# leeyevi/MV3D_TF

Hardware: AMD Instinct MI355X
Metric: KITTI-shape frames/sec (RPN+3-view ROI-pool+NMS) at 1/2/4/8 MI355X (higher is better)
Workload: dtype f32; 1 GPU; BASELINE configs[2] path-only: batch 2, 3 views; proposal_layer_3d TRAIN cfg (23104 BEV anchors, pre/post-NMS 12000/2000, NMS 0.7) + anchor_target + proposal_target (256 sampled ROIs in batch 0) + FV ROIs + RoiPool 7x7 fwd+bwd on BEV 76x76x512 / RGB 46x155x512 / FV 8x64x512; peaky scores; driven by the library's own mv3d_train_path (submit -> counts to the host -> numpy-global-RNG draws on the hel; batch_per_gpu=2, ring_batches=16, streams=8, launch=path, hipgraph=False, parallelism=frames/1, pmc_signature=train/b2/r256/peaky/pair-tiles-planned

## Files before the change

### include/mv3d_hip.h

```cpp
#ifndef MV3D_HIP_H
#define MV3D_HIP_H
#include <stddef.h>
#include <stdint.h>
#ifdef __cplusplus
extern "C" {
#endif

typedef enum {
    MV3D_OK = 0,
    MV3D_ERR_INVALID_ARG = 1,
    MV3D_ERR_WORKSPACE = 2,
    MV3D_ERR_HIP = 3,
    MV3D_ERR_ZERO_DIVISION = 4
} mv3d_status;

int mv3d_version(void);
const char *mv3d_status_string(int status);


size_t mv3d_nms_workspace_bytes(int max_boxes);
int mv3d_nms_device(const float *dets_dev, int n, double thresh, int max_keep,
                    int32_t *keep_dev, int32_t *num_keep_dev, int32_t *status_dev,
                    void *workspace, size_t workspace_bytes, void *stream);

// ... 103 lines not shown
                              const int32_t *disable_bg2_dev, int n_dis_bg2,
                              float *labels_dev, float *anchors_dev, float *anchors_3d_dev,
                              int32_t *n_anchors_dev, int anchors_cap,
                              void *workspace, size_t workspace_bytes, void *stream);

int mv3d_anchor_target_stage1_batch(int batch, int H, int W, const float *im_info_dev, const float *const *gt_bv_dev,
                                    const float *const *gt_3d_dev, const int *G, const mv3d_anchor_target_params *p,
                                    float *labels_dev, float *targets_dev, int32_t *const *counts_dev,
                                    uint8_t *const *fg_hi_dev, void *const *workspace, size_t workspace_bytes, void *stream);
int mv3d_anchor_target_stage2_batch(int batch, int H, int W, const mv3d_anchor_target_params *p,
                                    const int32_t *const *disable_fg_dev, const int *n_dis_fg,
                                    const int32_t *const *disable_bg1_dev, const int *n_dis_bg1,
                                    const int32_t *const *disable_bg2_dev, const int *n_dis_bg2, float *labels_dev,
                                    float *anchors_dev, float *anchors_3d_dev, int32_t *n_anchors_dev, int anchors_cap,
                                    void *const *workspace, size_t workspace_bytes, void *stream);

typedef struct {
    int32_t num_classes;
    int32_t frame_index;
    double fg_thresh;
    double bg_thresh_hi;
    double bg_thresh_lo;
} mv3d_proposal_target_params;

size_t mv3d_proposal_target_workspace_bytes(int num_rois, int G);
int mv3d_proposal_target_stage1(const float *rois_bv_dev, const float *rois_3d_dev, int num_rois,
                                const float *gt_bv_dev, const float *gt_3d_dev, int G,
                                const mv3d_proposal_target_params *p, int32_t *counts_dev,
                                void *workspace, size_t workspace_bytes, void *stream);
int mv3d_proposal_target_stage2(const float *rois_bv_dev, const float *rois_3d_dev, int num_rois,
// ... 43 lines not shown
int mv3d_legacy_permutation(void *mt19937_state, int32_t n, int32_t *out);
typedef struct {
    int32_t n_fg, n_bg, n_low;
    int32_t pt_n_fg, pt_n_bg;
    int32_t reserved0;
    const uint8_t *fg_alive;
} mv3d_draw_frame;
typedef struct {
    int32_t rpn_batchsize;
    int32_t rpn_num_fg;
    int32_t rois_per_image;
    int32_t roi_fg_max;
} mv3d_draw_params;
int mv3d_draw_training_subsamples(void *mt19937_state, int batch, const mv3d_draw_frame *frames, const mv3d_draw_params *par,
                                  int32_t *lists, size_t lists_cap, int32_t *sizes, int32_t *scratch, size_t scratch_cap);

typedef struct {
    int32_t batch, H, W, num_classes;
    int32_t proposal_cap;
    int32_t anchor_cap;
    int32_t roi_cap;
    int32_t max_gt;
    mv3d_proposal_params proposal;
    mv3d_anchor_target_params anchor;
    mv3d_proposal_target_params target;
    mv3d_draw_params draw;
} mv3d_train_path_config;
typedef struct {
    float *blob_bv, *blob_img, *blob_3d;
    int32_t *num_proposals;
// ... 11 lines not shown
    uint8_t *h_report; size_t h_report_row;
    int32_t *h_pt_counts;
    int32_t *h_num_proposals;
    int32_t *h_lists;
    int32_t *h_scratch; size_t scratch_cap;
} mv3d_train_path_slot;
typedef struct mv3d_train_path mv3d_train_path;
int mv3d_train_path_create(const mv3d_train_path_config *config, int depth, const mv3d_train_path_slot *slots, int helper_thread,
                           mv3d_train_path **out);
int mv3d_train_path_configure(mv3d_train_path *path, const mv3d_train_path_config *config);
int mv3d_train_path_submit(mv3d_train_path *path, int slot, const float *prob_dev, const float *pred_dev, const float *im_info_dev,
                           const float *calib_dev, const float *const *gt_bv_dev, const float *const *gt_3d_dev,
                           const float *const *gt_corners_dev, const int *G, void *mt19937_state, void *stream);
int mv3d_train_path_finish(mv3d_train_path *path, int slot, int32_t *rows_out, int32_t *num_proposals_out, int32_t *sizes_out);
int mv3d_train_path_host_seconds(mv3d_train_path *path, double *wait_s, double *draw_s);
void mv3d_train_path_destroy(mv3d_train_path *path);

int mv3d_gt_encode(const float *box_cam_dev, const double *cos_sin_dev, int num_objects, const float *inv_rot_dev,
                   const float *tr_velo_to_cam_dev, float *corners_cam_dev, float *corners_lidar_dev,
                   float *boxes_3d_dev, float *boxes_bv_dev, void *stream);

int mv3d_box_detect_tail(const float *rois_3d_dev, const float *bbox_pred_dev, int num_rois, int num_classes,
                         float *corners_dev, float *pred_cnr_r_dev, float *pred_bv_dev, float *pred_bv_r_dev,
                         void *stream);

typedef struct {
    int32_t num_classes;
    int32_t rows_per_frame;
    int32_t max_per_image;
    int32_t nms_strict_gt;
// ... 195 lines not shown
```

### mv3d_tf_amd/_lib.py

```python
import ctypes as C
import os

import torch

_HERE = os.path.dirname(os.path.abspath(__file__))
LIB_PATH = os.path.join(_HERE, "libmv3d_hip.so")

OK, ERR_INVALID_ARG, ERR_WORKSPACE, ERR_HIP, ERR_ZERO_DIVISION = 0, 1, 2, 3, 4


class ProposalParams(C.Structure):
    _fields_ = [("feat_stride", C.c_int32), ("pre_nms_topN", C.c_int32), ("post_nms_topN", C.c_int32),
                ("img_height", C.c_int32), ("img_width", C.c_int32), ("img_padding", C.c_int32),
                ("nms_strict_gt", C.c_int32), ("reserved0", C.c_int32), ("nms_thresh", C.c_double), ("min_size", C.c_double)]


class DetectPostParams(C.Structure):
    _fields_ = [("num_classes", C.c_int32), ("rows_per_frame", C.c_int32), ("max_per_image", C.c_int32),
                ("nms_strict_gt", C.c_int32), ("score_thresh", C.c_float), ("reserved0", C.c_int32), ("nms_thresh", C.c_double)]


class AnchorTargetParams(C.Structure):
    _fields_ = [("feat_stride", C.c_int32), ("clobber_positives", C.c_int32),
                ("negative_overlap", C.c_double), ("positive_overlap", C.c_double)]
# ... 109 lines not shown
    "mv3d_proposal_3d": (C.c_int, [_P, _P, C.c_int, C.c_int, C.c_int, _P, _P, C.POINTER(ProposalParams),
                                   _P, _P, _P, _P, _P, _P, C.c_size_t, _P]),
    "mv3d_roi_pool_forward": (C.c_int, [_P, C.c_float, C.c_int, C.c_int, C.c_int, C.c_int, C.c_int, C.c_int,
                                        C.c_int, _P, _P, _P, _P]),
    "mv3d_roi_pool_backward": (C.c_int, [_P, C.c_float, C.c_int, C.c_int, C.c_int, C.c_int, C.c_int, C.c_int,
                                         C.c_int, _P, _P, _P, _P]),
    "mv3d_anchor_target_workspace_bytes": (C.c_size_t, [C.c_int, C.c_int, C.c_int]),
    "mv3d_anchor_target_stage1": (C.c_int, [C.c_int, C.c_int, _P, _P, _P, C.c_int, C.POINTER(AnchorTargetParams),
                                            _P, _P, _P, _P, _P, C.c_size_t, _P]),
    "mv3d_anchor_target_stage2": (C.c_int, [C.c_int, C.c_int, C.POINTER(AnchorTargetParams), _P, C.c_int, _P,
                                            C.c_int, _P, C.c_int, _P, _P, _P, _P, C.c_int, _P, C.c_size_t, _P]),
    "mv3d_anchor_target_stage1_batch": (C.c_int, [C.c_int, C.c_int, C.c_int, _P, _P, _P, _P, C.POINTER(AnchorTargetParams), _P, _P, _P, _P,
                                                  _P, C.c_size_t, _P]),
    "mv3d_anchor_target_stage2_batch": (C.c_int, [C.c_int, C.c_int, C.c_int, C.POINTER(AnchorTargetParams), _P, _P, _P, _P, _P, _P, _P,
                                                  _P, _P, _P, C.c_int, _P, C.c_size_t, _P]),
    "mv3d_proposal_target_stage1_batch": (C.c_int, [C.c_int, _P, _P, _P, _P, _P, _P, _P, _P, _P, _P, _P]),
    "mv3d_proposal_target_stage2_batch": (C.c_int, [C.c_int, _P, _P, _P, _P, _P, _P, _P, _P, _P, _P, _P, _P, _P, _P, _P, _P, _P, _P, _P,
                                                    _P, _P, _P]),
    "mv3d_proposal_target_stage1_batch_devn": (C.c_int, [C.c_int, _P, _P, _P, _P, _P, _P, _P, _P, _P, _P, _P, _P]),
    "mv3d_proposal_target_stage2_batch_devn": (C.c_int, [C.c_int, _P, _P, _P, _P, _P, _P, _P, _P, _P, _P, _P, _P, _P, _P, _P, _P, _P, _P,
                                                         _P, _P, _P, _P, _P]),
    "mv3d_proposal_target_workspace_bytes": (C.c_size_t, [C.c_int, C.c_int]),
    "mv3d_proposal_target_stage1": (C.c_int, [_P, _P, C.c_int, _P, _P, C.c_int, C.POINTER(ProposalTargetParams), _P, _P,
                                              C.c_size_t, _P]),
    "mv3d_proposal_target_stage2": (C.c_int, [_P, _P, C.c_int, _P, _P, _P, C.c_int, _P, C.POINTER(ProposalTargetParams),
                                              _P, C.c_int, _P, C.c_int, _P, _P, _P, _P, _P, _P, C.c_size_t, _P]),
    "mv3d_point_cloud_2_top": (C.c_int, [_P, C.c_int, _P, _P]),
    "mv3d_point_cloud_2_top_shape": (C.c_int, [C.c_double] * 8 + [_P]),
    "mv3d_point_cloud_2_top_ranges": (C.c_int, [_P, C.c_int] + [C.c_double] * 8 + [_P, _P, _P]),
    "mv3d_box_detect_tail": (C.c_int, [_P, _P, C.c_int, C.c_int, _P, _P, _P, _P, _P]),
# ... 9 lines not shown
    "mv3d_roi_pool_forward_views": (C.c_int, [C.c_int, C.POINTER(RoiView), C.c_int, C.c_int, _P]),
    "mv3d_roi_pool_forward_views_cold": (C.c_int, [C.c_int, C.POINTER(RoiView), C.c_int, C.c_int, _P]),
    "mv3d_roi_pool_forward_views_half": (C.c_int, [C.c_int, C.POINTER(RoiView), C.c_int, C.c_int, C.c_int, C.c_int, _P]),
    "mv3d_roi_pool_backward_workspace_bytes": (C.c_size_t, [C.c_int, C.POINTER(RoiGradView), C.c_int, C.c_int]),
    "mv3d_roi_pool_backward_views": (C.c_int, [C.c_int, C.POINTER(RoiGradView), C.c_int, C.c_int, _P, C.c_size_t, _P]),
    "mv3d_roi_pool_pair_workspace_bytes": (C.c_size_t, [C.c_int, C.POINTER(RoiGradView), C.c_int, C.c_int]),
    "mv3d_roi_pool_forward_views_pair": (C.c_int, [C.c_int, C.POINTER(RoiView), C.c_int, C.c_int, C.c_int, _P]),
    "mv3d_roi_pool_backward_views_pair": (C.c_int, [C.c_int, C.POINTER(RoiGradView), C.c_int, C.c_int, _P, C.c_size_t, _P]),
    "mv3d_roi_pool_argmax_decode": (C.c_int, [C.c_int, C.POINTER(RoiView), C.c_int, C.c_int, C.POINTER(C.c_void_p), _P]),
    "mv3d_ROIPoolForwardLaucher": (C.c_int, [_P, C.c_float, C.c_int, C.c_int, C.c_int, C.c_int, C.c_int, C.c_int, _P, _P, _P, _P]),
    "mv3d_ROIPoolBackwardLaucher": (C.c_int, [_P, C.c_float, C.c_int, C.c_int, C.c_int, C.c_int, C.c_int, C.c_int, C.c_int, _P, _P, _P, _P]),
    "mv3d_rois_3d_to_fv": (C.c_int, [_P, C.c_int, _P, _P]),
    "mv3d_legacy_permutation": (C.c_int, [_P, C.c_int32, _P]),
    "mv3d_draw_training_subsamples": (C.c_int, [_P, C.c_int, C.POINTER(DrawFrame), C.POINTER(DrawParams), _P, C.c_size_t, _P, _P,
                                                C.c_size_t]),
    "mv3d_train_path_create": (C.c_int, [C.POINTER(TrainPathConfig), C.c_int, C.POINTER(TrainPathSlot), C.c_int, C.POINTER(C.c_void_p)]),
    "mv3d_train_path_configure": (C.c_int, [_P, C.POINTER(TrainPathConfig)]),
    "mv3d_train_path_submit": (C.c_int, [_P, C.c_int, _P, _P, _P, _P, _P, _P, _P, _P, _P, _P]),
    "mv3d_train_path_finish": (C.c_int, [_P, C.c_int, _P, _P, _P]),
    "mv3d_train_path_host_seconds": (C.c_int, [_P, C.POINTER(C.c_double), C.POINTER(C.c_double)]),
    "mv3d_train_path_destroy": (None, [_P]),
    "mv3d_gt_encode": (C.c_int, [_P, _P, C.c_int, _P, _P, _P, _P, _P, _P, _P]),
    "mv3d_conv3x3_f16": (C.c_int, [_P, _P, _P, _P, C.c_int, C.c_int, C.c_int, C.c_int, C.c_int, C.c_int, C.c_int, C.c_int, _P]),
    "mv3d_conv3x3_f32": (C.c_int, [_P, _P, _P, _P, C.c_int, C.c_int, C.c_int, C.c_int, C.c_int, C.c_int, C.c_int, _P]),
    "mv3d_maxpool2x2_f32": (C.c_int, [_P, _P, C.c_int, C.c_int, C.c_int, C.c_int, _P]),
    "mv3d_frame_nhwc_f32": (C.c_int, [_P, _P, C.c_int, C.c_int, C.c_int, C.c_int, C.c_int, _P]),
    "mv3d_conv3x3_bf16": (C.c_int, [_P, _P, _P, _P, C.c_int, C.c_int, C.c_int, C.c_int, C.c_int, C.c_int, C.c_int, C.c_int, _P]),
    "mv3d_maxpool2x2_bf16": (C.c_int, [_P, _P, C.c_int, C.c_int, C.c_int, C.c_int, _P]),
    "mv3d_frame_nhwc_bf16": (C.c_int, [_P, _P, C.c_int, C.c_int, C.c_int, C.c_int, C.c_int, _P]),
    "mv3d_conv3x3_wgrad_workspace_bytes": (C.c_size_t, [C.c_int, C.c_int, C.c_int, C.c_int, C.c_int]),
    "mv3d_conv3x3_wgrad_bf16": (C.c_int, [_P, _P, _P, _P, C.c_int, C.c_int, C.c_int, C.c_int, C.c_int, C.c_int, _P, C.c_size_t, _P]),
    "mv3d_conv3x3_wgrad_f32_workspace_bytes": (C.c_size_t, [C.c_int, C.c_int, C.c_int, C.c_int, C.c_int]),
    "mv3d_conv3x3_wgrad_f32": (C.c_int, [_P, _P, _P, _P, C.c_int, C.c_int, C.c_int, C.c_int, C.c_int, C.c_int, _P, C.c_size_t, _P]),
    "mv3d_conv3x3_pack_bf16": (C.c_int, [_P, _P, _P, C.c_int, C.c_int, C.c_int, _P]),
    "mv3d_conv3x3_gated_bf16": (C.c_int, [_P, _P, _P, _P, _P, C.c_int, C.c_int, C.c_int, C.c_int, C.c_int, _P]),
# ... 70 lines not shown
```

### mv3d_tf_amd/csrc/anchor_target.hip

```cpp
#include <math.h>
#include "common.h"

__constant__ int c_at_base[16] = {-19, -8, 20, 8, -5, -2, 5, 3, -8, -19, 8, 20, -2, -5, 3, 5};
#define AT_MAX_GT 1024

__device__ __forceinline__ double mv3d_log(double x)
{
    if (x != x || x < 0) return NAN;
    if (x == 0) return -INFINITY;
    if (isinf(x)) return x;
    int k;
    double m = frexp(x, &k);
    if (m < 0.70710678118654752440) { m *= 2.0; k -= 1; }
    const double s = (m - 1.0) / (m + 1.0);
    const double z = s * s;
    double p = 1.0 / 39;
#pragma unroll
    for (int d = 37; d >= 1; d -= 2) p = fma(p, z, 1.0 / d);
    const double LN2_HI = 6.93147180369123816490e-01, LN2_LO = 1.90821492927058770002e-10;
    const double lm = 2.0 * s * p;
    return fma((double)k, LN2_HI, fma((double)k, LN2_LO, lm));
}

__device__ __forceinline__ double iou_f64(double b0, double b1, double b2, double b3, double q0, double q1, double q2,
// ... 167 lines not shown
    if (blockIdx.x == gridDim.x - 1 && threadIdx.x == 0) {
        int32_t *counts = F.counts;
        counts[0] = tot[0]; counts[1] = tot[1]; counts[2] = tot[2]; counts[3] = tot[3];
        counts[4] = counts[5] = counts[6] = counts[7] = 0;
    }
}

__global__ __launch_bounds__(256) void at_disable_all_kernel(AtBatch bt)
{
    const AtFrame &F = bt.f[blockIdx.y];
    const int n1 = F.n_dis_fg, n2 = F.n_dis_bg1, n3 = F.n_dis_bg2;
    for (int t = blockIdx.x * blockDim.x + threadIdx.x; t < n1 + n2 + n3; t += gridDim.x * blockDim.x) {
        if (t < n1) F.d.labels[F.lists.fg[F.dis_fg[t]]] = -1.0f;
        else if (t < n1 + n2) F.d.labels[F.lists.bg[F.dis_bg1[t - n1]]] = -1.0f;
        else F.d.argmax[F.lists.low[F.dis_bg2[t - n1 - n2]]] = -1;
    }
}

__global__ __launch_bounds__(256) void at_emit_relabel_kernel(AtBatch bt)
{
    const AtFrame &F = bt.f[blockIdx.y];
    const AtDev &d = F.d;
    float *anchors = F.anchors, *anchors_3d = F.anchors_3d;
    const int cap = bt.cap;
    int tot[1];
    mv3d_grid_compact<1>(
        d.N,
        [&](int n, bool f[1]) { f[0] = anchors && (d.max_ov[n] >= 0.0) && (d.labels[n] != -1.0f); },
        [&](int, int r, int n) {
            if (r >= cap) return;
// ... 94 lines not shown
    hipLaunchKernelGGL(at_overlap_kernel, dim3(blocks, batch), dim3(256), 0, s, bt);
    hipLaunchKernelGGL(at_label_kernel, dim3(blocks, batch), dim3(256), 0, s, bt);
    hipLaunchKernelGGL(at_compact_kernel, dim3(L.ncwg, batch), dim3(256), 0, s, bt);
    return mv3d_launch_status();
}

extern "C" int mv3d_anchor_target_stage1(int H, int W, const float *im_info_dev, const float *gt_bv_dev,
                                         const float *gt_3d_dev, int G, const mv3d_anchor_target_params *p,
                                         float *labels_dev, float *targets_dev, int32_t *counts_dev, uint8_t *fg_hi_dev,
                                         void *workspace, size_t workspace_bytes, void *stream)
{
    return mv3d_anchor_target_stage1_batch(1, H, W, im_info_dev, &gt_bv_dev, &gt_3d_dev, &G, p, labels_dev, targets_dev,
                                           &counts_dev, &fg_hi_dev, &workspace, workspace_bytes, stream);
}

extern "C" int mv3d_anchor_target_stage2_batch(int batch, int H, int W, const mv3d_anchor_target_params *p,
                                               const int32_t *const *disable_fg_dev, const int *n_dis_fg,
                                               const int32_t *const *disable_bg1_dev, const int *n_dis_bg1,
                                               const int32_t *const *disable_bg2_dev, const int *n_dis_bg2, float *labels_dev,
                                               float *anchors_dev, float *anchors_3d_dev, int32_t *n_anchors_dev,
                                               int anchors_cap, void *const *workspace, size_t workspace_bytes, void *stream)
{
    if (batch <= 0 || batch > AT_MAX_BATCH || !p || !labels_dev || !workspace || !n_dis_fg || !n_dis_bg1 || !n_dis_bg2 ||
        !disable_fg_dev || !disable_bg1_dev || !disable_bg2_dev)
        return MV3D_ERR_INVALID_ARG;
    AtLayout L;
    if (!at_layout(H, W, 0, L)) return MV3D_ERR_INVALID_ARG;
    const bool emit = anchors_dev && anchors_3d_dev && n_anchors_dev;
    AtBatch bt = {};
    bt.cap = anchors_cap;
    int most = 0;
    for (int b = 0; b < batch; ++b) {
        if (n_dis_fg[b] < 0 || n_dis_bg1[b] < 0 || n_dis_bg2[b] < 0) return MV3D_ERR_INVALID_ARG;
        if ((n_dis_fg[b] && !disable_fg_dev[b]) || (n_dis_bg1[b] && !disable_bg1_dev[b]) || (n_dis_bg2[b] && !disable_bg2_dev[b]))
            return MV3D_ERR_INVALID_ARG;
        if (!workspace[b] || workspace_bytes < L.total || ((uintptr_t)workspace[b] % MV3D_ALIGN)) return MV3D_ERR_WORKSPACE;
        AtFrame &F = bt.f[b];
        at_frame(F, L, H, W, 0, p, (char *)workspace[b]);
        F.d.im_info = nullptr; F.d.gt_bv = nullptr; F.d.gt_3d = nullptr; F.d.targets = nullptr;
        F.d.labels = labels_dev + (size_t)b * L.N;
        F.dis_fg = disable_fg_dev[b]; F.dis_bg1 = disable_bg1_dev[b]; F.dis_bg2 = disable_bg2_dev[b];
        F.n_dis_fg = n_dis_fg[b]; F.n_dis_bg1 = n_dis_bg1[b]; F.n_dis_bg2 = n_dis_bg2[b];
        F.anchors = emit ? anchors_dev + (size_t)b * anchors_cap * 5 : nullptr;
        F.anchors_3d = emit ? anchors_3d_dev + (size_t)b * anchors_cap * 7 : nullptr;
        F.n_anchors = emit ? n_anchors_dev + b : nullptr;
        const int n = n_dis_fg[b] + n_dis_bg1[b] + n_dis_bg2[b];
        if (n > most) most = n;
    }
    hipStream_t s = (hipStream_t)stream;
    if (most > 0) hipLaunchKernelGGL(at_disable_all_kernel, dim3((most + 255) / 256, batch), dim3(256), 0, s, bt);
    hipLaunchKernelGGL(at_emit_relabel_kernel, dim3(L.ncwg, batch), dim3(256), 0, s, bt);
    return mv3d_launch_status();
}

extern "C" int mv3d_anchor_target_stage2(int H, int W, const mv3d_anchor_target_params *p,
                                         const int32_t *disable_fg_dev, int n_dis_fg, const int32_t *disable_bg1_dev,
                                         int n_dis_bg1, const int32_t *disable_bg2_dev, int n_dis_bg2, float *labels_dev,
                                         float *anchors_dev, float *anchors_3d_dev, int32_t *n_anchors_dev,
                                         int anchors_cap, void *workspace, size_t workspace_bytes, void *stream)
{
    return mv3d_anchor_target_stage2_batch(1, H, W, p, &disable_fg_dev, &n_dis_fg, &disable_bg1_dev, &n_dis_bg1, &disable_bg2_dev,
                                           &n_dis_bg2, labels_dev, anchors_dev, anchors_3d_dev, n_anchors_dev, anchors_cap,
                                           &workspace, workspace_bytes, stream);
}
```

### mv3d_tf_amd/csrc/legacy_rng.hip

```cpp
#include <stdint.h>
#include <string.h>
#include "../../include/mv3d_hip.h"

namespace {

constexpr int MT_N = 624, MT_M = 397;
struct MtState { uint32_t key[MT_N]; int pos; };

inline void mt_gen(MtState *s)
{
    uint32_t *k = s->key;
    int i;
    for (i = 0; i < MT_N - MT_M; ++i) {
        const uint32_t y = (k[i] & 0x80000000u) | (k[i + 1] & 0x7fffffffu);
        k[i] = k[i + MT_M] ^ (y >> 1) ^ ((y & 1u) ? 0x9908b0dfu : 0u);
    }
    for (; i < MT_N - 1; ++i) {
        const uint32_t y = (k[i] & 0x80000000u) | (k[i + 1] & 0x7fffffffu);
        k[i] = k[i + (MT_M - MT_N)] ^ (y >> 1) ^ ((y & 1u) ? 0x9908b0dfu : 0u);
    }
    const uint32_t y = (k[MT_N - 1] & 0x80000000u) | (k[0] & 0x7fffffffu);
    k[MT_N - 1] = k[MT_M - 1] ^ (y >> 1) ^ ((y & 1u) ? 0x9908b0dfu : 0u);
    s->pos = 0;
}
// ... 33 lines not shown
                t_lo = pos;
            }
            while (pos < MT_N && i > lo) {
                const uint32_t j = t[pos++] & mask;
                const bool ok = j <= (uint32_t)i;
                const uint32_t jj = ok ? j : (uint32_t)i;
                const int32_t a = x[i], b = x[jj];
                x[i] = b; x[jj] = a;
                i -= ok ? 1 : 0;
            }
        }
    }
    s->pos = pos;
}

}

extern "C" int mv3d_legacy_permutation(void *mt19937_state, int32_t n, int32_t *out)
{
    if (!mt19937_state || n < 0 || (n > 0 && !out)) return MV3D_ERR_INVALID_ARG;
    MtState *s = (MtState *)mt19937_state;
    if (s->pos < 0 || s->pos > MT_N) return MV3D_ERR_INVALID_ARG;
    permutation(s, n, out);
    return MV3D_OK;
}

extern "C" int mv3d_draw_training_subsamples(void *mt19937_state, int batch, const mv3d_draw_frame *frames,
                                             const mv3d_draw_params *par, int32_t *lists, size_t lists_cap, int32_t *sizes,
                                             int32_t *scratch, size_t scratch_cap)
{
// ... 31 lines not shown
            uint8_t *alive = (uint8_t *)scratch;
            for (int32_t i = 0; i < f.n_fg; ++i) alive[i] = f.fg_alive[i] ? 1 : 0;
            for (int32_t i = 0; i < sz[0]; ++i) alive[dis_fg[i]] = 0;
            for (int32_t i = 0; i < f.n_fg; ++i) n_pos += alive[i];
        }
        const int32_t num_bg2 = par->rpn_batchsize - n_pos;
        if (!emit(f.n_low, f.n_low - num_bg2, f.n_low > num_bg2, &sz[2])) return MV3D_ERR_WORKSPACE;
        const int32_t fg_n = par->roi_fg_max < f.pt_n_fg ? par->roi_fg_max : f.pt_n_fg;
        if (!emit(f.pt_n_fg, fg_n, f.pt_n_fg > 0, &sz[3])) return MV3D_ERR_WORKSPACE;
        const int32_t bg_room = par->rois_per_image - fg_n;
        const int32_t bg_n = bg_room < f.pt_n_bg ? bg_room : f.pt_n_bg;
        if (!emit(f.pt_n_bg, bg_n < 0 ? 0 : bg_n, f.pt_n_bg > 0, &sz[4])) return MV3D_ERR_WORKSPACE;
    }
    return MV3D_OK;
}
```

### mv3d_tf_amd/csrc/train_stream.hip

```cpp
#include <hip/hip_runtime.h>
#include <chrono>
#include <condition_variable>
#include <deque>
#include <mutex>
#include <new>
#include <thread>
#include <vector>
#include "common.h"
#include "../../include/mv3d_hip.h"

#define TP_MAX_BATCH 16

namespace {

enum SlotState { TP_IDLE = 0, TP_SUBMITTED = 1, TP_STAGED = 2 };

struct Slot {
    mv3d_train_path_slot buf;
    hipEvent_t ev = nullptr;
    int state = TP_IDLE, rc = MV3D_OK;
    hipStream_t stream = nullptr;
    void *mt = nullptr;
    const float *calib = nullptr;
    const float *gt_bv[TP_MAX_BATCH], *gt_3d[TP_MAX_BATCH], *gt_c[TP_MAX_BATCH];
    int G[TP_MAX_BATCH];
    int32_t sizes[5 * TP_MAX_BATCH], rows[TP_MAX_BATCH];
    std::vector<uint8_t> spill[TP_MAX_BATCH];
    float *p_bv[TP_MAX_BATCH], *p_3d[TP_MAX_BATCH];
    int32_t *p_num[TP_MAX_BATCH], *p_cnt[TP_MAX_BATCH], *a_cnt[TP_MAX_BATCH];
    uint8_t *a_fgh[TP_MAX_BATCH];
    void *a_ws[TP_MAX_BATCH], *p_ws[TP_MAX_BATCH];
    int p_cap[TP_MAX_BATCH];
    size_t p_wsz[TP_MAX_BATCH];
    uint8_t *dv_report = nullptr;
    int32_t *dv_pt_counts = nullptr, *dv_num_proposals = nullptr;
// ... 22 lines not shown
}

}

struct mv3d_train_path {
    mv3d_train_path_config cfg;
    mv3d_proposal_target_params tpar[TP_MAX_BATCH];
    int depth = 0, device = 0;
    std::vector<Slot> slots;
    bool threaded = false, stop = false;
    std::thread helper;
    std::mutex m;
    std::condition_variable cv_work, cv_done;
    std::deque<int> queue;
    double t_wait = 0.0, t_draw = 0.0;
};

namespace {

bool config_ok(const mv3d_train_path_config &c)
{
    return c.batch >= 1 && c.batch <= TP_MAX_BATCH && c.H > 0 && c.W > 0 && c.num_classes >= 1 && c.proposal_cap > 0 && c.anchor_cap > 0 &&
           c.roi_cap > 0 && c.max_gt > 0 && c.draw.rois_per_image <= c.roi_cap;
}

void set_params(mv3d_train_path *tp, const mv3d_train_path_config &c)
{
    tp->cfg = c;
    for (int b = 0; b < c.batch; ++b) {
        tp->tpar[b] = c.target;
// ... 32 lines not shown
        s.p_cap[b] = c.proposal_cap;
        s.p_wsz[b] = u.target_ws_bytes;
    }
}

#define TP_HIP(expr)                                 \
    do {                                             \
        if ((expr) != hipSuccess) return MV3D_ERR_HIP; \
    } while (0)

int host_stage(mv3d_train_path *tp, Slot &s)
{
    const mv3d_train_path_config &c = tp->cfg;
    const mv3d_train_path_slot &u = s.buf;
    const int B = c.batch, H = c.H, W = c.W;
    const auto t0 = std::chrono::steady_clock::now();
    TP_HIP(hipEventSynchronize(s.ev));
    const auto t1 = std::chrono::steady_clock::now();
    for (int b = 0; b < B; ++b)
        if (u.h_num_proposals[B + b] & MV3D_FLAG_ZERO_DIVISION) return MV3D_ERR_ZERO_DIVISION;
    mv3d_draw_frame fr[TP_MAX_BATCH];
    for (int b = 0; b < B; ++b) {
        const uint8_t *head = u.h_report + (size_t)b * u.h_report_row;
        const int32_t *cnt = (const int32_t *)head;
        fr[b].n_fg = cnt[1]; fr[b].n_bg = cnt[2]; fr[b].n_low = cnt[3];
        fr[b].pt_n_fg = u.h_pt_counts[4 * b + 1]; fr[b].pt_n_bg = u.h_pt_counts[4 * b + 2];
        fr[b].reserved0 = 0;
        if (cnt[1] < 0 || (size_t)cnt[1] > (size_t)4 * H * W) return MV3D_ERR_INVALID_ARG;
        if (32 + (size_t)cnt[1] <= u.h_report_row) {
            fr[b].fg_alive = head + 32;
        } else {
            s.spill[b].resize((size_t)cnt[1]);
            TP_HIP(hipMemcpyAsync(s.spill[b].data(), s.a_fgh[b], (size_t)cnt[1], hipMemcpyDeviceToHost, s.stream));
            TP_HIP(hipStreamSynchronize(s.stream));
            fr[b].fg_alive = s.spill[b].data();
        }
    }
    int rc = mv3d_draw_training_subsamples(s.mt, B, fr, &c.draw, u.h_lists, u.lists_cap, s.sizes, u.h_scratch, u.scratch_cap);
    const auto t2 = std::chrono::steady_clock::now();
    {
        std::lock_guard<std::mutex> g(tp->m);
        tp->t_wait += std::chrono::duration<double>(t1 - t0).count();
        tp->t_draw += std::chrono::duration<double>(t2 - t1).count();
    }
    if (rc != MV3D_OK) return rc;
    size_t off[5 * TP_MAX_BATCH + 1];
    off[0] = 0;
    for (int k = 0; k < 5 * B; ++k) off[k + 1] = off[k] + (size_t)s.sizes[k];
    const int32_t *const lists = u.lists;
    if (off[5 * B]) TP_HIP(hipMemcpyAsync(u.lists, u.h_lists, off[5 * B] * sizeof(int32_t), hipMemcpyHostToDevice, s.stream));
    const int32_t *lst[5][TP_MAX_BATCH];
    int cnt[5][TP_MAX_BATCH];
    for (int b = 0; b < B; ++b)
        for (int k = 0; k < 5; ++k) {
            cnt[k][b] = s.sizes[5 * b + k];
            lst[k][b] = cnt[k][b] ? lists + off[5 * b + k] : nullptr;
        }
    rc = mv3d_anchor_target_stage2_batch(B, H, W, &c.anchor, lst[0], cnt[0], lst[1], cnt[1], lst[2], cnt[2], u.rpn_labels, u.anchors,
                                         u.anchors_3d, u.n_anchors, c.anchor_cap, s.a_ws, u.anchor_ws_bytes, s.stream);
    if (rc != MV3D_OK) return rc;
    float *o_bev[TP_MAX_BATCH], *o_rgb[TP_MAX_BATCH], *o_fv[TP_MAX_BATCH], *o_3d[TP_MAX_BATCH], *o_tg[TP_MAX_BATCH];
    int32_t *o_lab[TP_MAX_BATCH];
    const float *cal[TP_MAX_BATCH];
    size_t row = 0;
    for (int b = 0; b < B; ++b) {
        const int S = cnt[3][b] + cnt[4][b];
        s.rows[b] = S;
        if (row + (size_t)S > (size_t)B * c.roi_cap) return MV3D_ERR_WORKSPACE;
        o_bev[b] = S ? u.rois_bev + row * 5 : nullptr;
        o_rgb[b] = S ? u.rois_rgb + row * 5 : nullptr;
        o_fv[b] = (S && u.rois_fv) ? u.rois_fv + row * 5 : nullptr;
        o_3d[b] = S ? u.rois_3d + row * 7 : nullptr;
        o_lab[b] = S ? u.labels + row : nullptr;
        o_tg[b] = S ? u.bbox_targets + row * 24 * c.num_classes : nullptr;
        cal[b] = s.calib + (size_t)b * 48;
        row += (size_t)S;
    }
    return mv3d_proposal_target_stage2_batch_devn(B, s.p_bv, s.p_3d, s.p_cap, s.p_num, s.gt_bv, s.gt_3d, s.gt_c, s.G, cal, tp->tpar, lst[3],
                                                  cnt[3], lst[4], cnt[4], o_bev, o_rgb, o_lab, o_tg, o_3d, u.rois_fv ? o_fv : nullptr, s.p_ws,
                                                  s.p_wsz, s.stream);
}

int host_stage_noexcept(mv3d_train_path *tp, Slot &s)
{
    try {
        return host_stage(tp, s);
    } catch (...) {
        return MV3D_ERR_WORKSPACE;
    }
}

void helper_main(mv3d_train_path *tp)
{
    (void)hipSetDevice(tp->device);
    for (;;) {
        int k;
        {
            std::unique_lock<std::mutex> g(tp->m);
            tp->cv_work.wait(g, [&] { return tp->stop || !tp->queue.empty(); });
            if (tp->queue.empty()) return;
            k = tp->queue.front();
            tp->queue.pop_front();
        }
        Slot &s = tp->slots[k];
        const int rc = host_stage_noexcept(tp, s);
        {
            std::lock_guard<std::mutex> g(tp->m);
            s.rc = rc;
            s.state = TP_STAGED;
        }
        tp->cv_done.notify_all();
    }
}

}

extern "C" int mv3d_train_path_create(const mv3d_train_path_config *config, int depth, const mv3d_train_path_slot *slots, int helper_thread,
                                      mv3d_train_path **out)
{
    if (!config || !slots || !out || depth < 1 || depth > 64 || !config_ok(*config)) return MV3D_ERR_INVALID_ARG;
    for (int k = 0; k < depth; ++k)
        if (!slot_ok(*config, slots[k])) return MV3D_ERR_INVALID_ARG;
    mv3d_train_path *tp = new (std::nothrow) mv3d_train_path();
    if (!tp) return MV3D_ERR_HIP;
    set_params(tp, *config);
    tp->depth = depth;
    if (hipGetDevice(&tp->device) != hipSuccess) { delete tp; return MV3D_ERR_HIP; }
    try {
        tp->slots.resize((size_t)depth);
    } catch (...) {
        delete tp;
        return MV3D_ERR_HIP;
    }
    for (int k = 0; k < depth; ++k) {
        Slot &s = tp->slots[k];
        s.buf = slots[k];
        slot_tables(tp->cfg, s);
        {
            void *d0 = nullptr, *d1 = nullptr, *d2 = nullptr;
            const bool mapped = hipHostGetDevicePointer(&d0, s.buf.h_report, 0) == hipSuccess && hipHostGetDevicePointer(&d1, s.buf.h_pt_counts, 0) == hipSuccess &&
                                hipHostGetDevicePointer(&d2, s.buf.h_num_proposals, 0) == hipSuccess && d0 && d1 && d2;
            (void)hipGetLastError();
            if (mapped && s.buf.h_report_row % 16 == 0 && (uintptr_t)d0 % 16 == 0 && (uintptr_t)s.buf.report % 16 == 0 && !tp_force_copies()) {
                s.dv_report = (uint8_t *)d0; s.dv_pt_counts = (int32_t *)d1; s.dv_num_proposals = (int32_t *)d2;
// ... 117 lines not shown
    std::lock_guard<std::mutex> g(tp->m);
    s.state = TP_IDLE;
    return rc;
}

extern "C" int mv3d_train_path_host_seconds(mv3d_train_path *tp, double *wait_s, double *draw_s)
{
    if (!tp) return MV3D_ERR_INVALID_ARG;
    std::lock_guard<std::mutex> g(tp->m);
    if (wait_s) *wait_s = tp->t_wait;
    if (draw_s) *draw_s = tp->t_draw;
    tp->t_wait = tp->t_draw = 0.0;
    return MV3D_OK;
}

extern "C" void mv3d_train_path_destroy(mv3d_train_path *tp)
{
    if (!tp) return;
    if (tp->threaded) {
        {
            std::lock_guard<std::mutex> g(tp->m);
            tp->stop = true;
        }
        tp->cv_work.notify_all();
        tp->helper.join();
    }
    for (Slot &s : tp->slots)
        if (s.ev) (void)hipEventDestroy(s.ev);
    delete tp;
}
// ... 1 lines not shown
```

### mv3d_tf_amd/train_path.py

```python
import ctypes as C

import numpy as np
import numpy.random as npr
import torch

from . import ops
from ._lib import AnchorTargetParams, DrawParams, ProposalTargetParams, TrainPathConfig, TrainPathSlot, check, lib
from .fast_rcnn.config import cfg

_HEAD = 4096


def draw_subsamples_host(head, n_fg_flags_fetch, N):
    T = cfg.TRAIN
    n_inside, n_fg, n_bg, n_low = (int(v) for v in head[:16].view(np.int32))
    num_fg = int(T.RPN_FG_FRACTION * T.RPN_BATCHSIZE)
    dis_fg = npr.permutation(n_fg)[:n_fg - num_fg] if n_fg > num_fg else None
    num_bg = T.RPN_BATCHSIZE - min(n_fg, num_fg)
    dis_bg1 = npr.permutation(n_bg)[:n_bg - num_bg] if n_bg > num_bg else None
    n_pos = 0
    if n_fg:
        alive = (head[32:32 + n_fg] if 32 + n_fg <= len(head) else n_fg_flags_fetch()[:n_fg]).astype(bool)
        if dis_fg is not None:
            alive[dis_fg] = False
# ... 149 lines not shown
        if h:
            lib().mv3d_train_path_destroy(h)

    def __del__(self):
        try:
            self.close()
        except Exception:
            pass

    @property
    def host_seconds(self):
        w, d = C.c_double(), C.c_double()
        check(lib().mv3d_train_path_host_seconds(self._h, C.byref(w), C.byref(d)), "mv3d_train_path_host_seconds")
        return w.value, d.value

    def finish(self, s):
        s.busy = False
        check(lib().mv3d_train_path_finish(self._h, s.index, s.rows_c, s.nprop_c, s.sizes_c), "mv3d_train_path_finish")
        S = list(s.rows_c)
        St = sum(S)
        return {"rpn_labels": s.rpn_labels, "rpn_targets": s.rpn_targets, "anchors": s.anchors, "anchors_3d": s.anchors_3d,
                "n_anchors": s.n_anchors, "rois": {k: v[:St] for k, v in s.rois.items()}, "rois_3d": s.rois_3d[:St],
                "labels": s.labels[:St], "bbox_targets": s.bbox_targets[:St], "S": S,
                "num_proposals": list(s.nprop_c), "proposals": s.prop, "stream": s.stream, "draw_sizes": list(s.sizes_c)}
```

Baseline: 16940 frames/s.

## Draw background subsample keep-sets as bitmaps with tail-only Fisher-Yates shuffle

```diff
diff --git a/include/mv3d_hip.h b/include/mv3d_hip.h
--- a/include/mv3d_hip.h
+++ b/include/mv3d_hip.h
@@ -141,6 +141,12 @@
                                     const int32_t *const *disable_bg2_dev, const int *n_dis_bg2, float *labels_dev,
                                     float *anchors_dev, float *anchors_3d_dev, int32_t *n_anchors_dev, int anchors_cap,
                                     void *const *workspace, size_t workspace_bytes, void *stream);
+int mv3d_anchor_target_stage2_keep_batch(int batch, int H, int W, const mv3d_anchor_target_params *p,
+                                         const int32_t *const *disable_fg_dev, const int *n_dis_fg,
+                                         const int32_t *const *keep_bg1_dev, const int *n_bg,
+                                         const int32_t *const *keep_bg2_dev, const int *n_low, float *labels_dev,
+                                         float *anchors_dev, float *anchors_3d_dev, int32_t *n_anchors_dev, int anchors_cap,
+                                         void *const *workspace, size_t workspace_bytes, void *stream);
 
 typedef struct {
     int32_t num_classes;
@@ -214,6 +220,10 @@
 } mv3d_draw_params;
 int mv3d_draw_training_subsamples(void *mt19937_state, int batch, const mv3d_draw_frame *frames, const mv3d_draw_params *par,
                                   int32_t *lists, size_t lists_cap, int32_t *sizes, int32_t *scratch, size_t scratch_cap);
+int mv3d_legacy_permutation_keep(void *mt19937_state, int32_t n, int32_t k, int32_t *identity, int32_t *bitmap);
+int mv3d_draw_training_keep_sets(void *mt19937_state, int batch, const mv3d_draw_frame *frames, const mv3d_draw_params *par,
+                                 int32_t *lists, size_t lists_cap, int32_t *sizes, int32_t *words, int32_t *scratch,
+                                 size_t scratch_cap, int32_t *identity, size_t identity_cap);
 
 typedef struct {
     int32_t batch, H, W, num_classes;
@@ -255,6 +265,7 @@
                            const float *const *gt_corners_dev, const int *G, void *mt19937_state, void *stream);
 int mv3d_train_path_finish(mv3d_train_path *path, int slot, int32_t *rows_out, int32_t *num_proposals_out, int32_t *sizes_out);
 int mv3d_train_path_host_seconds(mv3d_train_path *path, double *wait_s, double *draw_s);
+int mv3d_train_path_host_profile(mv3d_train_path *path, double *seconds, long long *batches);
 void mv3d_train_path_destroy(mv3d_train_path *path);
 
 int mv3d_gt_encode(const float *box_cam_dev, const double *cos_sin_dev, int num_objects, const float *inv_rot_dev,
diff --git a/mv3d_tf_amd/_lib.py b/mv3d_tf_amd/_lib.py
--- a/mv3d_tf_amd/_lib.py
+++ b/mv3d_tf_amd/_lib.py
@@ -147,6 +147,8 @@
                                                   _P, C.c_size_t, _P]),
     "mv3d_anchor_target_stage2_batch": (C.c_int, [C.c_int, C.c_int, C.c_int, C.POINTER(AnchorTargetParams), _P, _P, _P, _P, _P, _P, _P,
                                                   _P, _P, _P, C.c_int, _P, C.c_size_t, _P]),
+    "mv3d_anchor_target_stage2_keep_batch": (C.c_int, [C.c_int, C.c_int, C.c_int, C.POINTER(AnchorTargetParams), _P, _P, _P, _P, _P, _P, _P,
+                                                       _P, _P, _P, C.c_int, _P, C.c_size_t, _P]),
     "mv3d_proposal_target_stage1_batch": (C.c_int, [C.c_int, _P, _P, _P, _P, _P, _P, _P, _P, _P, _P, _P]),
     "mv3d_proposal_target_stage2_batch": (C.c_int, [C.c_int, _P, _P, _P, _P, _P, _P, _P, _P, _P, _P, _P, _P, _P, _P, _P, _P, _P, _P, _P,
                                                     _P, _P, _P]),
@@ -186,11 +188,15 @@
     "mv3d_legacy_permutation": (C.c_int, [_P, C.c_int32, _P]),
     "mv3d_draw_training_subsamples": (C.c_int, [_P, C.c_int, C.POINTER(DrawFrame), C.POINTER(DrawParams), _P, C.c_size_t, _P, _P,
                                                 C.c_size_t]),
+    "mv3d_legacy_permutation_keep": (C.c_int, [_P, C.c_int32, C.c_int32, _P, _P]),
+    "mv3d_draw_training_keep_sets": (C.c_int, [_P, C.c_int, C.POINTER(DrawFrame), C.POINTER(DrawParams), _P, C.c_size_t, _P, _P, _P,
+                                               C.c_size_t, _P, C.c_size_t]),
     "mv3d_train_path_create": (C.c_int, [C.POINTER(TrainPathConfig), C.c_int, C.POINTER(TrainPathSlot), C.c_int, C.POINTER(C.c_void_p)]),
     "mv3d_train_path_configure": (C.c_int, [_P, C.POINTER(TrainPathConfig)]),
     "mv3d_train_path_submit": (C.c_int, [_P, C.c_int, _P, _P, _P, _P, _P, _P, _P, _P, _P, _P]),
     "mv3d_train_path_finish": (C.c_int, [_P, C.c_int, _P, _P, _P]),
     "mv3d_train_path_host_seconds": (C.c_int, [_P, C.POINTER(C.c_double), C.POINTER(C.c_double)]),
+    "mv3d_train_path_host_profile": (C.c_int, [_P, C.POINTER(C.c_double), C.POINTER(C.c_longlong)]),
     "mv3d_train_path_destroy": (None, [_P]),
     "mv3d_gt_encode": (C.c_int, [_P, _P, C.c_int, _P, _P, _P, _P, _P, _P, _P]),
     "mv3d_conv3x3_f16": (C.c_int, [_P, _P, _P, _P, C.c_int, C.c_int, C.c_int, C.c_int, C.c_int, C.c_int, C.c_int, C.c_int, _P]),
diff --git a/mv3d_tf_amd/csrc/anchor_target.hip b/mv3d_tf_amd/csrc/anchor_target.hip
--- a/mv3d_tf_amd/csrc/anchor_target.hip
+++ b/mv3d_tf_amd/csrc/anchor_target.hip
@@ -205,6 +205,18 @@
         if (t < n1) F.d.labels[F.lists.fg[F.dis_fg[t]]] = -1.0f;
         else if (t < n1 + n2) F.d.labels[F.lists.bg[F.dis_bg1[t - n1]]] = -1.0f;
         else F.d.argmax[F.lists.low[F.dis_bg2[t - n1 - n2]]] = -1;
+    }
+}
+
+__global__ __launch_bounds__(256) void at_disable_keep_kernel(AtBatch bt)
+{
+    const AtFrame &F = bt.f[blockIdx.y];
+    const int n1 = F.n_dis_fg, n2 = F.n_dis_bg1, n3 = F.n_dis_bg2;
+    const int most = max(n1, max(n2, n3));
+    for (int t = blockIdx.x * blockDim.x + threadIdx.x; t < most; t += gridDim.x * blockDim.x) {
+        if (t < n1) F.d.labels[F.lists.fg[F.dis_fg[t]]] = -1.0f;
+        if (t < n2 && !(((uint32_t)F.dis_bg1[t >> 5] >> (t & 31)) & 1u)) F.d.labels[F.lists.bg[t]] = -1.0f;
+        if (t < n3 && !(((uint32_t)F.dis_bg2[t >> 5] >> (t & 31)) & 1u)) F.d.argmax[F.lists.low[t]] = -1;
     }
 }
 
@@ -329,15 +341,13 @@
                                            &counts_dev, &fg_hi_dev, &workspace, workspace_bytes, stream);
 }
 
-extern "C" int mv3d_anchor_target_stage2_batch(int batch, int H, int W, const mv3d_anchor_target_params *p,
-                                               const int32_t *const *disable_fg_dev, const int *n_dis_fg,
-                                               const int32_t *const *disable_bg1_dev, const int *n_dis_bg1,
-                                               const int32_t *const *disable_bg2_dev, const int *n_dis_bg2, float *labels_dev,
-                                               float *anchors_dev, float *anchors_3d_dev, int32_t *n_anchors_dev,
-                                               int anchors_cap, void *const *workspace, size_t workspace_bytes, void *stream)
-{
-    if (batch <= 0 || batch > AT_MAX_BATCH || !p || !labels_dev || !workspace || !n_dis_fg || !n_dis_bg1 || !n_dis_bg2 ||
-        !disable_fg_dev || !disable_bg1_dev || !disable_bg2_dev)
+static int at_stage2(bool keep, int batch, int H, int W, const mv3d_anchor_target_params *p, const int32_t *const *disable_fg_dev,
+                     const int *n_dis_fg, const int32_t *const *bg1_dev, const int *n_bg1, const int32_t *const *bg2_dev, const int *n_bg2,
+                     float *labels_dev, float *anchors_dev, float *anchors_3d_dev, int32_t *n_anchors_dev, int anchors_cap,
+                     void *const *workspace, size_t workspace_bytes, void *stream)
+{
+    if (batch <= 0 || batch > AT_MAX_BATCH || !p || !labels_dev || !workspace || !n_dis_fg || !n_bg1 || !n_bg2 || !disable_fg_dev ||
+        !bg1_dev || !bg2_dev)
         return MV3D_ERR_INVALID_ARG;
     AtLayout L;
     if (!at_layout(H, W, 0, L)) return MV3D_ERR_INVALID_ARG;
@@ -346,26 +356,50 @@
     bt.cap = anchors_cap;
     int most = 0;
     for (int b = 0; b < batch; ++b) {
-        if (n_dis_fg[b] < 0 || n_dis_bg1[b] < 0 || n_dis_bg2[b] < 0) return MV3D_ERR_INVALID_ARG;
-        if ((n_dis_fg[b] && !disable_fg_dev[b]) || (n_dis_bg1[b] && !disable_bg1_dev[b]) || (n_dis_bg2[b] && !disable_bg2_dev[b]))
-            return MV3D_ERR_INVALID_ARG;
+        if (n_dis_fg[b] < 0 || n_bg1[b] < 0 || n_bg2[b] < 0) return MV3D_ERR_INVALID_ARG;
+        if ((n_dis_fg[b] && !disable_fg_dev[b]) || (n_bg1[b] && !bg1_dev[b]) || (n_bg2[b] && !bg2_dev[b])) return MV3D_ERR_INVALID_ARG;
+        if (keep && (n_bg1[b] > L.N || n_bg2[b] > L.N)) return MV3D_ERR_INVALID_ARG;
         if (!workspace[b] || workspace_bytes < L.total || ((uintptr_t)workspace[b] % MV3D_ALIGN)) return MV3D_ERR_WORKSPACE;
         AtFrame &F = bt.f[b];
         at_frame(F, L, H, W, 0, p, (char *)workspace[b]);
         F.d.im_info = nullptr; F.d.gt_bv = nullptr; F.d.gt_3d = nullptr; F.d.targets = nullptr;
         F.d.labels = labels_dev + (size_t)b * L.N;
-        F.dis_fg = disable_fg_dev[b]; F.dis_bg1 = disable_bg1_dev[b]; F.dis_bg2 = disable_bg2_dev[b];
-        F.n_dis_fg = n_dis_fg[b]; F.n_dis_bg1 = n_dis_bg1[b]; F.n_dis_bg2 = n_dis_bg2[b];
+        F.dis_fg = disable_fg_dev[b]; F.dis_bg1 = bg1_dev[b]; F.dis_bg2 = bg2_dev[b];
+        F.n_dis_fg = n_dis_fg[b]; F.n_dis_bg1 = n_bg1[b]; F.n_dis_bg2 = n_bg2[b];
         F.anchors = emit ? anchors_dev + (size_t)b * anchors_cap * 5 : nullptr;
         F.anchors_3d = emit ? anchors_3d_dev + (size_t)b * anchors_cap * 7 : nullptr;
         F.n_anchors = emit ? n_anchors_dev + b : nullptr;
-        const int n = n_dis_fg[b] + n_dis_bg1[b] + n_dis_bg2[b];
+        const int big = n_bg1[b] > n_bg2[b] ? n_bg1[b] : n_bg2[b];
+        const int n = keep ? (n_dis_fg[b] > big ? n_dis_fg[b] : big) : n_dis_fg[b] + n_bg1[b] + n_bg2[b];
         if (n > most) most = n;
     }
     hipStream_t s = (hipStream_t)stream;
-    if (most > 0) hipLaunchKernelGGL(at_disable_all_kernel, dim3((most + 255) / 256, batch), dim3(256), 0, s, bt);
+    if (most > 0 && keep) hipLaunchKernelGGL(at_disable_keep_kernel, dim3((most + 255) / 256, batch), dim3(256), 0, s, bt);
+    else if (most > 0) hipLaunchKernelGGL(at_disable_all_kernel, dim3((most + 255) / 256, batch), dim3(256), 0, s, bt);
     hipLaunchKernelGGL(at_emit_relabel_kernel, dim3(L.ncwg, batch), dim3(256), 0, s, bt);
     return mv3d_launch_status();
+}
+
+extern "C" int mv3d_anchor_target_stage2_batch(int batch, int H, int W, const mv3d_anchor_target_params *p,
+                                               const int32_t *const *disable_fg_dev, const int *n_dis_fg,
+                                               const int32_t *const *disable_bg1_dev, const int *n_dis_bg1,
+                                               const int32_t *const *disable_bg2_dev, const int *n_dis_bg2, float *labels_dev,
+                                               float *anchors_dev, float *anchors_3d_dev, int32_t *n_anchors_dev,
+                                               int anchors_cap, void *const *workspace, size_t workspace_bytes, void *stream)
+{
+    return at_stage2(false, batch, H, W, p, disable_fg_dev, n_dis_fg, disable_bg1_dev, n_dis_bg1, disable_bg2_dev, n_dis_bg2, labels_dev,
+                     anchors_dev, anchors_3d_dev, n_anchors_dev, anchors_cap, workspace, workspace_bytes, stream);
+}
+
+extern "C" int mv3d_anchor_target_stage2_keep_batch(int batch, int H, int W, const mv3d_anchor_target_params *p,
+                                                    const int32_t *const *disable_fg_dev, const int *n_dis_fg,
+                                                    const int32_t *const *keep_bg1_dev, const int *n_bg,
+                                                    const int32_t *const *keep_bg2_dev, const int *n_low, float *labels_dev,
+                                                    float *anchors_dev, float *anchors_3d_dev, int32_t *n_anchors_dev,
+                                                    int anchors_cap, void *const *workspace, size_t workspace_bytes, void *stream)
+{
+    return at_stage2(true, batch, H, W, p, disable_fg_dev, n_dis_fg, keep_bg1_dev, n_bg, keep_bg2_dev, n_low, labels_dev, anchors_dev,
+                     anchors_3d_dev, n_anchors_dev, anchors_cap, workspace, workspace_bytes, stream);
 }
 
 extern "C" int mv3d_anchor_target_stage2(int H, int W, const mv3d_anchor_target_params *p,
diff --git a/mv3d_tf_amd/csrc/legacy_rng.hip b/mv3d_tf_amd/csrc/legacy_rng.hip
--- a/mv3d_tf_amd/csrc/legacy_rng.hip
+++ b/mv3d_tf_amd/csrc/legacy_rng.hip
@@ -71,6 +71,87 @@
     s->pos = pos;
 }
 
+inline void temper_from(const MtState *s, int pos, uint32_t *t)
+{
+    for (int k = pos; k < MT_N; ++k) {
+        uint32_t y = s->key[k];
+        y ^= (y >> 11);
+        y ^= (y << 7) & 0x9d2c5680u;
+        y ^= (y << 15) & 0xefc60000u;
+        y ^= (y >> 18);
+        t[k] = y;
+    }
+}
+
+constexpr int KEEP_CH = 32;
+void permutation_keep(MtState *s, int32_t n, int32_t k, int32_t *x, uint32_t *bits)
+{
+    for (int32_t w = 0; w < (n + 31) / 32; ++w) bits[w] = 0;
+    if (n <= 0) return;
+    const int32_t stop = n - k;
+    const int32_t swap_lo = stop > 1 ? stop : 1;
+    int32_t i = n - 1;
+    int pos = s->pos;
+    uint32_t t[MT_N];
+    int t_lo = MT_N;
+    while (i >= swap_lo) {
+        const uint32_t mask = 0xffffffffu >> __builtin_clz((uint32_t)i);
+        const int32_t seg = (int32_t)(mask >> 1), lo = seg > swap_lo - 1 ? seg : swap_lo - 1;
+        while (i > lo) {
+            if (pos == MT_N) { mt_gen(s); pos = 0; t_lo = MT_N; }
+            if (t_lo > pos) { temper_from(s, pos, t); t_lo = pos; }
+            while (pos < MT_N && i > lo) {
+                const uint32_t j = t[pos++] & mask;
+                const bool ok = j <= (uint32_t)i;
+                const uint32_t jj = ok ? j : (uint32_t)i;
+                const int32_t a = x[i], b = x[jj];
+                x[i] = b; x[jj] = a;
+                i -= ok ? 1 : 0;
+            }
+        }
+    }
+    for (int32_t p = stop; p < n; ++p) {
+        const int32_t v = x[p];
+        bits[v >> 5] |= 1u << (v & 31);
+        if (v < stop) x[v] = v;
+    }
+    for (int32_t p = stop; p < n; ++p) x[p] = p;
+    while (i >= 1) {
+        const uint32_t mask = 0xffffffffu >> __builtin_clz((uint32_t)i);
+        const int32_t lo = (int32_t)(mask >> 1);
+        while (i > lo) {
+            if (pos == MT_N) { mt_gen(s); pos = 0; t_lo = MT_N; }
+            if (t_lo > pos) { temper_from(s, pos, t); t_lo = pos; }
+            while (pos + KEEP_CH <= MT_N && i - KEEP_CH >= lo) {
+                const uint32_t hi = (uint32_t)i, sure = (uint32_t)(i - KEEP_CH);
+                int n_sure = 0, n_hi = 0;
+                for (int c = 0; c < KEEP_CH; ++c) {
+                    const uint32_t w = t[pos + c] & mask;
+                    n_sure += w <= sure ? 1 : 0;
+                    n_hi += w <= hi ? 1 : 0;
+                }
+                if (n_sure == n_hi) {
+                    i -= n_sure;
+                } else {
+                    for (int c = 0; c < KEEP_CH; ++c) i -= (t[pos + c] & mask) <= (uint32_t)i ? 1 : 0;
+                }
+                pos += KEEP_CH;
+            }
+            while (pos < MT_N && i > lo) i -= (t[pos++] & mask) <= (uint32_t)i ? 1 : 0;
+        }
+    }
+    s->pos = pos;
+}
+
+}
+
+extern "C" int mv3d_legacy_permutation_keep(void *mt19937_state, int32_t n, int32_t k, int32_t *identity, int32_t *bitmap)
+{
+    if (!mt19937_state || n < 0 || k < 0 || k > n || (n > 0 && (!identity || !bitmap))) return MV3D_ERR_INVALID_ARG;
+    MtState *s = (MtState *)mt19937_state;
+    if (s->pos < 0 || s->pos > MT_N) return MV3D_ERR_INVALID_ARG;
+    permutation_keep(s, n, k, identity, (uint32_t *)bitmap);
+    return MV3D_OK;
 }
 
 extern "C" int mv3d_legacy_permutation(void *mt19937_state, int32_t n, int32_t *out)
@@ -132,3 +213,65 @@
     }
     return MV3D_OK;
 }
+
+extern "C" int mv3d_draw_training_keep_sets(void *mt19937_state, int batch, const mv3d_draw_frame *frames, const mv3d_draw_params *par,
+                                            int32_t *lists, size_t lists_cap, int32_t *sizes, int32_t *words, int32_t *scratch,
+                                            size_t scratch_cap, int32_t *identity, size_t identity_cap)
+{
+    if (!mt19937_state || batch <= 0 || !frames || !par || !lists || !sizes || !words || !scratch || !identity) return MV3D_ERR_INVALID_ARG;
+    MtState *s = (MtState *)mt19937_state;
+    if (s->pos < 0 || s->pos > MT_N) return MV3D_ERR_INVALID_ARG;
+    size_t o = 0;
+    auto emit = [&](int32_t n, int32_t take, bool draw, int32_t *size_out, int32_t *words_out) -> bool {
+        *size_out = *words_out = 0;
+        if (!draw) return true;
+        if (n < 0 || (size_t)n > scratch_cap || take < 0 || take > n || o + (size_t)take > lists_cap) return false;
+        if (take == n) {
+            permutation(s, n, lists + o);
+        } else {
+            permutation(s, n, scratch);
+            memcpy(lists + o, scratch, (size_t)take * sizeof(int32_t));
+        }
+        *size_out = *words_out = take;
+        o += (size_t)take;
+        return true;
+    };
+    auto emit_keep = [&](int32_t n, int32_t keep, bool draw, int32_t *size_out, int32_t *words_out) -> bool {
+        *size_out = *words_out = 0;
+        if (!draw) return true;
+        const size_t w = ((size_t)(n < 0 ? 0 : n) + 31) / 32;
+        if (n < 0 || (size_t)n > identity_cap || keep < 0 || keep > n || o + w > lists_cap) return false;
+        permutation_keep(s, n, keep, identity, (uint32_t *)(lists + o));
+        *size_out = n - keep;
+        *words_out = (int32_t)w;
+        o += w;
+        return true;
+    };
+    for (int b = 0; b < batch; ++b) {
+        const mv3d_draw_frame &f = frames[b];
+        int32_t *sz = sizes + 5 * b, *wd = words + 5 * b;
+        if (f.n_fg < 0 || f.n_bg < 0 || f.n_low < 0 || f.pt_n_fg < 0 || f.pt_n_bg < 0 || (f.n_fg > 0 && !f.fg_alive))
+            return MV3D_ERR_INVALID_ARG;
+        const int32_t num_fg = par->rpn_num_fg;
+        const int32_t *dis_fg = lists + o;
+        if (!emit(f.n_fg, f.n_fg - num_fg, f.n_fg > num_fg, &sz[0], &wd[0])) return MV3D_ERR_WORKSPACE;
+        const int32_t num_bg = par->rpn_batchsize - (f.n_fg < num_fg ? f.n_fg : num_fg);
+        if (!emit_keep(f.n_bg, num_bg, f.n_bg > num_bg, &sz[1], &wd[1])) return MV3D_ERR_WORKSPACE;
+        int32_t n_pos = 0;
+        if (f.n_fg > 0) {
+            if ((size_t)f.n_fg > scratch_cap) return MV3D_ERR_WORKSPACE;
+            uint8_t *alive = (uint8_t *)scratch;
+            for (int32_t i = 0; i < f.n_fg; ++i) alive[i] = f.fg_alive[i] ? 1 : 0;
+            for (int32_t i = 0; i < sz[0]; ++i) alive[dis_fg[i]] = 0;
+            for (int32_t i = 0; i < f.n_fg; ++i) n_pos += alive[i];
+        }
+        const int32_t num_bg2 = par->rpn_batchsize - n_pos;
+        if (!emit_keep(f.n_low, num_bg2, f.n_low > num_bg2, &sz[2], &wd[2])) return MV3D_ERR_WORKSPACE;
+        const int32_t fg_n = par->roi_fg_max < f.pt_n_fg ? par->roi_fg_max : f.pt_n_fg;
+        if (!emit(f.pt_n_fg, fg_n, f.pt_n_fg > 0, &sz[3], &wd[3])) return MV3D_ERR_WORKSPACE;
+        const int32_t bg_room = par->rois_per_image - fg_n;
+        const int32_t bg_n = bg_room < f.pt_n_bg ? bg_room : f.pt_n_bg;
+        if (!emit(f.pt_n_bg, bg_n < 0 ? 0 : bg_n, f.pt_n_bg > 0, &sz[4], &wd[4])) return MV3D_ERR_WORKSPACE;
+    }
+    return MV3D_OK;
+}
diff --git a/mv3d_tf_amd/csrc/train_stream.hip b/mv3d_tf_amd/csrc/train_stream.hip
--- a/mv3d_tf_amd/csrc/train_stream.hip
+++ b/mv3d_tf_amd/csrc/train_stream.hip
@@ -19,6 +19,7 @@
     mv3d_train_path_slot buf;
     hipEvent_t ev = nullptr;
     int state = TP_IDLE, rc = MV3D_OK;
+    double t_wait_draw = 0.0;
     hipStream_t stream = nullptr;
     void *mt = nullptr;
     const float *calib = nullptr;
@@ -71,6 +72,9 @@
     std::condition_variable cv_work, cv_done;
     std::deque<int> queue;
     double t_wait = 0.0, t_draw = 0.0;
+    std::vector<int32_t> identity;
+    double prof[4] = {0.0, 0.0, 0.0, 0.0};
+    long long prof_batches = 0;
 };
 
 namespace {
@@ -133,6 +137,7 @@
     const mv3d_train_path_config &c = tp->cfg;
     const mv3d_train_path_slot &u = s.buf;
     const int B = c.batch, H = c.H, W = c.W;
+    s.t_wait_draw = 0.0;
     const auto t0 = std::chrono::steady_clock::now();
     TP_HIP(hipEventSynchronize(s.ev));
     const auto t1 = std::chrono::steady_clock::now();
@@ -155,17 +160,22 @@
             fr[b].fg_alive = s.spill[b].data();
         }
     }
-    int rc = mv3d_draw_training_subsamples(s.mt, B, fr, &c.draw, u.h_lists, u.lists_cap, s.sizes, u.h_scratch, u.scratch_cap);
+    int32_t words[5 * TP_MAX_BATCH];
+    int rc = mv3d_draw_training_keep_sets(s.mt, B, fr, &c.draw, u.h_lists, u.lists_cap, s.sizes, words, u.h_scratch, u.scratch_cap,
+                                          tp->identity.data(), tp->identity.size());
     const auto t2 = std::chrono::steady_clock::now();
     {
         std::lock_guard<std::mutex> g(tp->m);
         tp->t_wait += std::chrono::duration<double>(t1 - t0).count();
         tp->t_draw += std::chrono::duration<double>(t2 - t1).count();
+        tp->prof[0] += std::chrono::duration<double>(t1 - t0).count();
+        tp->prof[1] += std::chrono::duration<double>(t2 - t1).count();
+        s.t_wait_draw = std::chrono::duration<double>(t2 - t0).count();
     }
     if (rc != MV3D_OK) return rc;
     size_t off[5 * TP_MAX_BATCH + 1];
     off[0] = 0;
-    for (int k = 0; k < 5 * B; ++k) off[k + 1] = off[k] + (size_t)s.sizes[k];
+    for (int k = 0; k < 5 * B; ++k) off[k + 1] = off[k] + (size_t)words[k];
     const int32_t *const lists = u.lists;
     if (off[5 * B]) TP_HIP(hipMemcpyAsync(u.lists, u.h_lists, off[5 * B] * sizeof(int32_t), hipMemcpyHostToDevice, s.stream));
     const int32_t *lst[5][TP_MAX_BATCH];
@@ -173,10 +183,14 @@
     for (int b = 0; b < B; ++b)
         for (int k = 0; k < 5; ++k) {
             cnt[k][b] = s.sizes[5 * b + k];
-            lst[k][b] = cnt[k][b] ? lists + off[5 * b + k] : nullptr;
-        }
-    rc = mv3d_anchor_target_stage2_batch(B, H, W, &c.anchor, lst[0], cnt[0], lst[1], cnt[1], lst[2], cnt[2], u.rpn_labels, u.anchors,
-                                         u.anchors_3d, u.n_anchors, c.anchor_cap, s.a_ws, u.anchor_ws_bytes, s.stream);
+            lst[k][b] = words[5 * b + k] ? lists + off[5 * b + k] : nullptr;
+        }
+    for (int b = 0; b < B; ++b) {
+        cnt[1][b] = words[5 * b + 1] ? fr[b].n_bg : 0;
+        cnt[2][b] = words[5 * b + 2] ? fr[b].n_low : 0;
+    }
+    rc = mv3d_anchor_target_stage2_keep_batch(B, H, W, &c.anchor, lst[0], cnt[0], lst[1], cnt[1], lst[2], cnt[2], u.rpn_labels, u.anchors,
+                                              u.anchors_3d, u.n_anchors, c.anchor_cap, s.a_ws, u.anchor_ws_bytes, s.stream);
     if (rc != MV3D_OK) return rc;
     float *o_bev[TP_MAX_BATCH], *o_rgb[TP_MAX_BATCH], *o_fv[TP_MAX_BATCH], *o_3d[TP_MAX_BATCH], *o_tg[TP_MAX_BATCH];
     int32_t *o_lab[TP_MAX_BATCH];
@@ -202,11 +216,18 @@
 
 int host_stage_noexcept(mv3d_train_path *tp, Slot &s)
 {
+    const auto t0 = std::chrono::steady_clock::now();
+    int rc;
     try {
-        return host_stage(tp, s);
+        rc = host_stage(tp, s);
     } catch (...) {
-        return MV3D_ERR_WORKSPACE;
-    }
+        rc = MV3D_ERR_WORKSPACE;
+    }
+    const double all = std::chrono::duration<double>(std::chrono::steady_clock::now() - t0).count();
+    std::lock_guard<std::mutex> g(tp->m);
+    tp->prof[2] += all - s.t_wait_draw;
+    tp->prof_batches += 1;
+    return rc;
 }
 
 void helper_main(mv3d_train_path *tp)
@@ -215,8 +236,10 @@
     for (;;) {
         int k;
         {
+            const auto t0 = std::chrono::steady_clock::now();
             std::unique_lock<std::mutex> g(tp->m);
             tp->cv_work.wait(g, [&] { return tp->stop || !tp->queue.empty(); });
+            tp->prof[3] += std::chrono::duration<double>(std::chrono::steady_clock::now() - t0).count();
             if (tp->queue.empty()) return;
             k = tp->queue.front();
             tp->queue.pop_front();
@@ -247,6 +270,8 @@
     if (hipGetDevice(&tp->device) != hipSuccess) { delete tp; return MV3D_ERR_HIP; }
     try {
         tp->slots.resize((size_t)depth);
+        tp->identity.resize((size_t)4 * config->H * config->W);
+        for (size_t i = 0; i < tp->identity.size(); ++i) tp->identity[i] = (int32_t)i;
     } catch (...) {
         delete tp;
         return MV3D_ERR_HIP;
@@ -394,6 +419,16 @@
     return MV3D_OK;
 }
 
+extern "C" int mv3d_train_path_host_profile(mv3d_train_path *tp, double *seconds, long long *batches)
+{
+    if (!tp || !seconds) return MV3D_ERR_INVALID_ARG;
+    std::lock_guard<std::mutex> g(tp->m);
+    for (int k = 0; k < 4; ++k) { seconds[k] = tp->prof[k]; tp->prof[k] = 0.0; }
+    if (batches) *batches = tp->prof_batches;
+    tp->prof_batches = 0;
+    return MV3D_OK;
+}
+
 extern "C" void mv3d_train_path_destroy(mv3d_train_path *tp)
 {
     if (!tp) return;
diff --git a/mv3d_tf_amd/train_path.py b/mv3d_tf_amd/train_path.py
--- a/mv3d_tf_amd/train_path.py
+++ b/mv3d_tf_amd/train_path.py
@@ -187,6 +187,11 @@
         check(lib().mv3d_train_path_host_seconds(self._h, C.byref(w), C.byref(d)), "mv3d_train_path_host_seconds")
         return w.value, d.value
 
+    def host_profile(self):
+        sec, nb = (C.c_double * 4)(), C.c_longlong()
+        check(lib().mv3d_train_path_host_profile(self._h, sec, C.byref(nb)), "mv3d_train_path_host_profile")
+        return dict(zip(("wait_stage1", "draw", "upload_enqueue", "idle"), sec)), nb.value
+
     def finish(self, s):
         s.busy = False
         check(lib().mv3d_train_path_finish(self._h, s.index, s.rows_c, s.nprop_c, s.sizes_c), "mv3d_train_path_finish")
```

Result: no change. 17180 frames/s (median of 4 runs) (+1.4%).
